# iosefa/obia

Measured on AMD Instinct MI355X. Metric: Mpixel/s (SLIC+zonal feats) on 16384²×8-band; achieved HBM GB/s fraction, higher is better.
Workload: dtype f32

## Files before the change

obia_amd/_lib.py:

```python
import ctypes
import os
import subprocess

import numpy as np

_CSRC = os.path.join(os.path.dirname(os.path.abspath(__file__)), "csrc")
LIB_PATH = os.environ.get("OBIA_HIP_LIB") or os.path.join(_CSRC, "libobia_hip.so")

OBIA_OK = 0
MASK_SEEDS_CHUNK = 1024
E_INVALID, E_HIP, E_NOMEM, E_UNSUPPORTED, E_EMPTY, E_NONFINITE = -1, -2, -3, -4, -5, -6


class SlicParams(ctypes.Structure):
    _fields_ = [("compactness", ctypes.c_double), ("min_size_factor", ctypes.c_double),
                ("max_size_factor", ctypes.c_double), ("n_segments", ctypes.c_int32),
                ("max_num_iter", ctypes.c_int32), ("convert2lab", ctypes.c_int32),
                ("enforce_connectivity", ctypes.c_int32), ("slic_zero", ctypes.c_int32),
                ("start_label", ctypes.c_int32), ("normalize_bands", ctypes.c_int32),
                ("exit_on_fixed_point", ctypes.c_int32), ("reserved", ctypes.c_int32),
                ("sigma_zyx", ctypes.c_double * 3), ("spacing_zyx", ctypes.c_double * 3)]


class SlicSeeds(ctypes.Structure):
# ... 140 lines not shown


def last_error():
    return load().obia_last_error().decode("utf-8", "replace")


def check(rc):
    if rc == OBIA_OK:
        return
    msg = last_error()
    if rc in (E_INVALID, E_EMPTY, E_NONFINITE):
        raise ValueError(msg)
    if rc == E_UNSUPPORTED:
        raise NotImplementedError(msg)
    if rc == E_NOMEM:
        raise MemoryError(msg)
    raise RuntimeError(f"obia_hip error {rc}: {msg}")


class Context:

    def __init__(self, device=0, stream=None):
        lib = load()
        if stream is None:
            self._h = lib.obia_create(int(device))
        else:
            self._h = lib.obia_create_on_stream(int(device), ctypes.c_void_p(int(stream)))
        if not self._h:
            raise RuntimeError(f"obia_create failed: {last_error()} (obia_amd needs an AMD GPU; there is no CPU path)")
        self.device = int(device)

    @property
    def handle(self):
        return self._h

    def close(self):
        if getattr(self, "_h", None):
            load().obia_destroy(self._h)
            self._h = None

    def __del__(self):
        try:
            self.close()
        except Exception:
            pass

    def set_profiling(self, on):
        check(load().obia_set_profiling(self._h, int(on)))

    def timing(self):
        lib = load()
        names = ["assign_ms", "sweeps", "features_ms", "connectivity_ms", "zonal_ms", "total_ms", "prepass_ms", "assign_px",
                 "prepass_px", "assign_store_px", "assign_busy_ms", "prepass_busy_ms", "batch_repeats",
                 "prepass_shared_px", "feature_fused_px"]
        return {n: lib.obia_last_timing(self._h, i) for i, n in enumerate(names)}

    def workspace_bytes(self):
        return int(load().obia_workspace_bytes(self._h))


_default_ctx = {}


def default_context(device=0):
    ctx = _default_ctx.get(device)
    if ctx is None:
        ctx = _default_ctx[device] = Context(device)
    return ctx


def np_ptr(a):
    return None if a is None else ctypes.c_void_p(a.ctypes.data)


def mask_bytes(mask, device=None):
    import torch
    m = torch.as_tensor(mask, device=device)
    if m.dtype == torch.bool:
        m = m.contiguous().view(torch.uint8)
    elif m.dtype != torch.uint8:
        m = (m != 0).view(torch.uint8)
    return m.contiguous()
```

obia_amd/csrc/common.hpp:

```cpp
#pragma once
#include <hip/hip_runtime.h>
#include <cstdint>
#include <cstdio>
#include <cstring>
#include <string>
#include <vector>

#include "../../include/obia_hip.h"

namespace obia {

void set_error(const char *fmt, ...);

#define OBIA_HIP_TRY(expr)                                                                       \
    do {                                                                                         \
        hipError_t e__ = (expr);                                                                 \
        if (e__ != hipSuccess) {                                                                 \
            obia::set_error("%s:%d: %s -> %s", __FILE__, __LINE__, #expr, hipGetErrorString(e__)); \
            return OBIA_E_HIP;                                                                   \
        }                                                                                        \
    } while (0)

#define OBIA_TRY(expr)            \
    do {                          \
        int rc__ = (expr);        \
        if (rc__ != OBIA_OK) return rc__; \
    } while (0)

class Arena {
  public:
    ~Arena() { release(); }
    void *alloc(size_t bytes);
    template <typename T> T *get(size_t n) { return static_cast<T *>(alloc(n * sizeof(T))); }
    void reset();
    void release();
    struct Mark { size_t block, used, total; };
    Mark mark() const;
    void rewind(const Mark &m);
    size_t capacity() const;
    bool failed() const { return failed_; }

  private:
    struct Block { char *p; size_t size; size_t used; };
    std::vector<Block> blocks_;
    size_t high_water_ = 0, cur_total_ = 0, cur_ = 0;
    bool failed_ = false;
};

struct Timing {
    double assign_ms = 0, prepass_ms = 0, feat_ms = 0, cc_ms = 0, zonal_ms = 0, total_ms = 0;
    double assign_px = 0, prepass_px = 0;
    double prepass_shared_px = 0;
    double assign_store_px = 0;
    double feat_fused_px = 0;
    int sweeps = 0;
    int batch_repeats = 0;
    double assign_busy_ms = 0, prepass_busy_ms = 0;
};

}

struct obia_ctx {
    int device = 0;
    hipStream_t stream = nullptr;
    bool own_stream = false;
    obia::Arena arena;
    void *pinned = nullptr;
    size_t pinned_bytes = 0;
    unsigned long long *defer_buf = nullptr;
    bool defer_pending = false;
    double defer_shared_px = 0;
    int32_t *cc_visited = nullptr;
    size_t cc_visited_px = 0;
    bool cc_visited_dirty = false;
    char *up_buf = nullptr;
    size_t up_bytes = 0, up_used = 0;
    int profiling = 0;
    obia::Timing timing;
    struct Span { int kind; hipEvent_t a, b; };
    std::vector<Span> spans;
    std::vector<hipEvent_t> event_pool;
    size_t events_used = 0;
    hipStream_t side = nullptr;
    hipEvent_t aux_fork = nullptr, aux_join = nullptr;
};

namespace obia {

enum TimeKind { T_ASSIGN = 0, T_FEAT = 2, T_CC = 3, T_ZONAL = 4, T_TOTAL = 5, T_PREPASS = 6 };

struct ScopedSpan {
    obia_ctx *ctx; bool on; size_t idx;
    ScopedSpan(obia_ctx *c, int kind);
    ~ScopedSpan();
};
struct KernelSpan {
    hipEvent_t a = nullptr, b = nullptr;
    KernelSpan(obia_ctx *c, int kind);
};
void begin_timing(obia_ctx *ctx);
void resolve_timing(obia_ctx *ctx);

int read_back(obia_ctx *ctx, void *host_dst, const void *dev_src, size_t bytes);
int upload_async(obia_ctx *ctx, void *dev_dst, const void *host_src, size_t bytes);
int side_stream(obia_ctx *ctx);
void debug_sync(obia_ctx *ctx, const char *stage);

static inline int cdiv(long long a, long long b) { return (int)((a + b - 1) / b); }

#if defined(__HIPCC__)
typedef float obia_v4f __attribute__((ext_vector_type(4)));
__device__ __forceinline__ float4 ld_stream_f4(const void *p) {
    const obia_v4f t = __builtin_nontemporal_load(reinterpret_cast<const obia_v4f *>(p));
    return make_float4(t.x, t.y, t.z, t.w);
}
#endif

}
```

obia_amd/csrc/context.cpp:

```cpp
#include "common.hpp"

#include <algorithm>
#include <cstdlib>
#include <utility>

#include <cstdarg>

namespace obia {

static thread_local std::string g_last_error;

void set_error(const char *fmt, ...) {
    char buf[1024];
    va_list ap;
    va_start(ap, fmt);
    vsnprintf(buf, sizeof(buf), fmt, ap);
    va_end(ap);
    g_last_error = buf;
}

void *Arena::alloc(size_t bytes) {
    bytes = (bytes + 255) & ~size_t(255);
    if (bytes == 0) bytes = 256;
    for (; cur_ < blocks_.size(); ++cur_) {
// ... 42 lines not shown
}

void Arena::reset() {
    failed_ = false;
    cur_total_ = 0;
    cur_ = 0;
    if (blocks_.size() > 1) {
        size_t total = 0;
        for (auto &b : blocks_) total += b.size;
        for (auto &b : blocks_) (void)hipFree(b.p);
        blocks_.clear();
        void *p = nullptr;
        if (hipMalloc(&p, high_water_ + (high_water_ >> 3)) == hipSuccess) blocks_.push_back(Block{static_cast<char *>(p), high_water_ + (high_water_ >> 3), 0});
        (void)total;
    } else if (!blocks_.empty()) {
        blocks_[0].used = 0;
    }
}

void Arena::release() {
    for (auto &b : blocks_) (void)hipFree(b.p);
    blocks_.clear();
}

size_t Arena::capacity() const {
    size_t t = 0;
    for (auto &b : blocks_) t += b.size;
    return t;
}

static hipEvent_t get_event(obia_ctx *ctx) {
    if (ctx->events_used == ctx->event_pool.size()) {
        hipEvent_t e = nullptr;
        (void)hipEventCreate(&e);
        ctx->event_pool.push_back(e);
    }
    return ctx->event_pool[ctx->events_used++];
}

ScopedSpan::ScopedSpan(obia_ctx *c, int kind) : ctx(c), on(c->profiling == 1 || (c->profiling == 2 && kind == T_ASSIGN)), idx(0) {
    if (!on) return;
    obia_ctx::Span s{kind, get_event(ctx), get_event(ctx)};
    (void)hipEventRecord(s.a, ctx->stream);
    idx = ctx->spans.size();
    ctx->spans.push_back(s);
}
ScopedSpan::~ScopedSpan() {
    if (on) (void)hipEventRecord(ctx->spans[idx].b, ctx->stream);
}

int side_stream(obia_ctx *ctx) {
    if (!ctx->aux_fork) OBIA_HIP_TRY(hipEventCreateWithFlags(&ctx->aux_fork, hipEventDisableTiming));
    if (!ctx->aux_join) OBIA_HIP_TRY(hipEventCreateWithFlags(&ctx->aux_join, hipEventDisableTiming));
    if (!ctx->side) OBIA_HIP_TRY(hipStreamCreateWithFlags(&ctx->side, hipStreamNonBlocking));
    return OBIA_OK;
}

KernelSpan::KernelSpan(obia_ctx *c, int kind) {
    if (!(c->profiling == 1 || (c->profiling == 2 && kind == T_ASSIGN))) return;
    a = get_event(c);
    b = get_event(c);
    c->spans.push_back(obia_ctx::Span{kind, a, b});
}

void begin_timing(obia_ctx *ctx) {
    ctx->spans.clear();
    ctx->events_used = 0;
    ctx->timing = Timing();
}

void resolve_timing(obia_ctx *ctx) {
    if (!ctx->profiling) return;
    (void)hipStreamSynchronize(ctx->stream);
    std::vector<std::pair<double, double>> iv[2];
    hipEvent_t ref = nullptr;
    for (auto &s : ctx->spans) {
        float ms = 0;
        if (hipEventElapsedTime(&ms, s.a, s.b) != hipSuccess) { (void)hipGetLastError(); continue; }
        if (s.kind == T_ASSIGN || s.kind == T_PREPASS) {
            if (!ref) ref = s.a;
            float end = 0;
            if (hipEventElapsedTime(&end, ref, s.b) == hipSuccess) iv[s.kind == T_ASSIGN ? 0 : 1].emplace_back((double)end - ms, (double)end);
            else (void)hipGetLastError();
        }
        switch (s.kind) {
            case T_ASSIGN: ctx->timing.assign_ms += ms; ctx->timing.sweeps += 1; break;
            case T_FEAT: ctx->timing.feat_ms += ms; break;
            case T_CC: ctx->timing.cc_ms += ms; break;
            case T_ZONAL: ctx->timing.zonal_ms += ms; break;
            case T_TOTAL: ctx->timing.total_ms += ms; break;
            case T_PREPASS: ctx->timing.prepass_ms += ms; break;
            default: break;
        }
    }
    for (int c = 0; c < 2; ++c) {
        std::sort(iv[c].begin(), iv[c].end());
        double busy = 0, lo = 0, hi = -1;
        for (auto &x : iv[c]) {
            if (hi < lo || x.first > hi) { if (hi > lo) busy += hi - lo; lo = x.first; hi = x.second; }
            else if (x.second > hi) hi = x.second;
        }
        if (hi > lo) busy += hi - lo;
        (c == 0 ? ctx->timing.assign_busy_ms : ctx->timing.prepass_busy_ms) += busy;
    }
    ctx->spans.clear();
}
// ... 53 lines not shown
using namespace obia;

extern "C" {

int obia_abi_version(void) { return OBIA_ABI_VERSION; }

const char *obia_last_error(void) { return g_last_error.c_str(); }

static obia_ctx *create_impl(int device_id, void *stream, bool own) {
    int n = 0;
    if (hipGetDeviceCount(&n) != hipSuccess || n <= 0) {
        set_error("no HIP device available");
        return nullptr;
    }
    if (device_id < 0 || device_id >= n) {
        set_error("device_id %d out of range (%d devices)", device_id, n);
        return nullptr;
    }
    if (hipSetDevice(device_id) != hipSuccess) {
        set_error("hipSetDevice(%d) failed", device_id);
        return nullptr;
    }
    obia_ctx *ctx = new obia_ctx();
    ctx->device = device_id;
    if (own) {
        if (hipStreamCreateWithFlags(&ctx->stream, hipStreamNonBlocking) != hipSuccess) {
            set_error("hipStreamCreate failed");
            delete ctx;
            return nullptr;
        }
        ctx->own_stream = true;
    } else {
        ctx->stream = static_cast<hipStream_t>(stream);
    }
    return ctx;
}

obia_ctx *obia_create(int device_id) { return create_impl(device_id, nullptr, true); }
obia_ctx *obia_create_on_stream(int device_id, void *hip_stream) { return create_impl(device_id, hip_stream, false); }

void obia_destroy(obia_ctx *ctx) {
    if (!ctx) return;
    (void)hipSetDevice(ctx->device);
    (void)hipStreamSynchronize(ctx->stream);
    ctx->arena.release();
    if (ctx->up_buf) (void)hipHostFree(ctx->up_buf);
    if (ctx->pinned) (void)hipHostFree(ctx->pinned);
    if (ctx->defer_buf) (void)hipHostFree(ctx->defer_buf);
    if (ctx->cc_visited) (void)hipFree(ctx->cc_visited);
    for (auto e : ctx->event_pool) (void)hipEventDestroy(e);
    if (ctx->side) (void)hipStreamDestroy(ctx->side);
    if (ctx->aux_fork) (void)hipEventDestroy(ctx->aux_fork);
    if (ctx->aux_join) (void)hipEventDestroy(ctx->aux_join);
    if (ctx->own_stream) (void)hipStreamDestroy(ctx->stream);
    delete ctx;
}

int obia_synchronize(obia_ctx *ctx) {
    if (!ctx) { set_error("null context"); return OBIA_E_INVALID; }
    OBIA_HIP_TRY(hipStreamSynchronize(ctx->stream));
    return OBIA_OK;
}

int64_t obia_workspace_bytes(obia_ctx *ctx) { return ctx ? (int64_t)ctx->arena.capacity() : 0; }

void obia_slic_default_params(obia_slic_params *p) {
    if (!p) return;
    p->n_segments = 100;
    p->compactness = 10.0;
    p->max_num_iter = 10;
    p->convert2lab = -1;
    p->enforce_connectivity = 1;
    p->min_size_factor = 0.5;
    p->max_size_factor = 3.0;
    p->slic_zero = 0;
    p->start_label = 1;
    p->normalize_bands = 0;
    p->exit_on_fixed_point = 0;
    p->reserved = 0;
    p->sigma_zyx[0] = p->sigma_zyx[1] = p->sigma_zyx[2] = 0.0;
    p->spacing_zyx[0] = p->spacing_zyx[1] = p->spacing_zyx[2] = 1.0;
}

int obia_set_profiling(obia_ctx *ctx, int enabled) {
    if (!ctx) { set_error("null context"); return OBIA_E_INVALID; }
    ctx->profiling = enabled < 0 ? 0 : (enabled > 2 ? 1 : enabled);
    return OBIA_OK;
}

double obia_last_timing(obia_ctx *ctx, int what) {
    if (!ctx) return -1.0;
    switch (what) {
        case 0: return ctx->timing.assign_ms;
        case 1: return (double)ctx->timing.sweeps;
        case 2: return ctx->timing.feat_ms;
        case 3: return ctx->timing.cc_ms;
        case 4: return ctx->timing.zonal_ms;
        case 5: return ctx->timing.total_ms;
        case 6: return ctx->timing.prepass_ms;
        case 7: return ctx->timing.assign_px;
        case 8: return ctx->timing.prepass_px;
        case 9: return ctx->timing.assign_store_px;
        case 10: return ctx->timing.assign_busy_ms;
        case 11: return ctx->timing.prepass_busy_ms;
        case 12: return (double)ctx->timing.batch_repeats;
        case 13: return ctx->timing.prepass_shared_px;
        case 14: return ctx->timing.feat_fused_px;
        default: return -1.0;
    }
}

}
```

obia_amd/csrc/slic_sweep.hip:

```cpp
#include "slic.hpp"
#include "slic_features.hpp"

#include <type_traits>
#include <hip/hip_ext.h>

#include <cstdlib>

namespace obia {

#ifdef OBIA_STAMP
__device__ unsigned long long g_tl[65536 * 4 * 24];
#define STAMP_DECL unsigned long long st_t = clock64(), st_t0 = st_t, st_r0 = __builtin_amdgcn_s_memrealtime(), st_acc[12] = {0, 0, 0, 0, 0, 0, 0, 0, 0, 0, 0, 0}, st_cnt[6] = {0, 0, 0, 0, 0, 0};
#define STAMP_COUNT(i, v) st_cnt[i] += (v);
#define STAMP(i) { const unsigned long long st_n = clock64(); st_acc[i] += st_n - st_t; st_t = st_n; }
#ifndef OBIA_STAMP_KIND
#define OBIA_STAMP_KIND 0
#endif
#define STAMP_FLUSH if (accumulate && (LEAN ? 1 : 0) == OBIA_STAMP_KIND && (threadIdx.x & 63) == 0 && gtile < 65536) { unsigned long long *st_o = g_tl + ((size_t)gtile * 4 + (threadIdx.x >> 6)) * 24; for (int st_i = 0; st_i < 12; ++st_i) st_o[st_i] = st_acc[st_i]; st_o[12] = st_t0; st_o[13] = clock64(); st_o[14] = st_r0; st_o[15] = __builtin_amdgcn_s_memrealtime(); for (int st_i = 0; st_i < 6; ++st_i) st_o[16 + st_i] = st_cnt[st_i]; }
#else
#define STAMP_DECL
#define STAMP(i)
#define STAMP_COUNT(i, v)
#define STAMP_FLUSH
#endif
// ... 86 lines not shown
        if (live) a[q] = 0ull;
        const unsigned long long nq = __shfl(aq, gl0 + CP);
        const unsigned long long syq = __shfl(aq, gl0 + CP + 1);
        const unsigned long long sxq = __shfl(aq, gl0 + CP + 2);
        const float fn = (float)nq;
        cy = (float)syq / fn;
        cx = (float)sxq / fn;
        bool mq = false;
        if (live && q < CP) {
            const float sum = (float)((double)(long long)aq * inv_fscale);
            const float v = sum / fn;
            mq = __float_as_uint(v) != __float_as_uint(oldc);
            rec[CENT_REC + q] = v;
        }
        const unsigned long long mb = __ballot(mq);
        const unsigned long long gmask = (G == 64) ? ~0ull : (((1ull << G) - 1ull) << gl0);
        moved = (mb & gmask) != 0ull;
        moved |= __float_as_uint(cy) != __float_as_uint(old_cy) || __float_as_uint(cx) != __float_as_uint(old_cx);
    }
    if (!live || q != 0) return;
    const float mdc = slic_zero ? ((first || slic_zero == 2) ? 1.0f : rec[7]) : 0.0f;
    if (bin_stamp && moved && !first && old_cy == old_cy && old_cx == old_cx) {
        int oby = (int)(old_cy / (float)P.sy), obx = (int)(old_cx / (float)P.sx);
        oby = oby < 0 ? 0 : (oby >= P.ncy ? P.ncy - 1 : oby);
        obx = obx < 0 ? 0 : (obx >= P.ncx ? P.ncx - 1 : obx);
        bin_stamp[P.cell_off + oby * P.ncx + obx] = sweep_id;
    }
    float4 *hrec = reinterpret_cast<float4 *>(rec);
    if (!(cy == cy) || !(cx == cx)) {
        hrec[0] = make_float4(cy, cx, 0.0f, 0.0f);
        hrec[1] = make_float4(0.0f, 0.0f, __int_as_float(-1), mdc);
        return;
    }
    float fy0 = cy - (float)(2 * P.sy); fy0 = (0.0f > fy0) ? 0.0f : fy0;
    float fy1 = (cy + (float)(2 * P.sy)) + 1.0f; fy1 = ((float)P.H < fy1) ? (float)P.H : fy1;
    float fx0 = cx - (float)(2 * P.sx); fx0 = (0.0f > fx0) ? 0.0f : fx0;
    float fx1 = (cx + (float)(2 * P.sx)) + 1.0f; fx1 = ((float)P.W < fx1) ? (float)P.W : fx1;
    int by = (int)(cy / (float)P.sy), bx = (int)(cx / (float)P.sx);
    by = by < 0 ? 0 : (by >= P.ncy ? P.ncy - 1 : by);
    bx = bx < 0 ? 0 : (bx >= P.ncx ? P.ncx - 1 : bx);
    const int link = atomicExch(&head[P.cell_off + by * P.ncx + bx], k);
    hrec[0] = make_float4(cy, cx, __int_as_float((int)fy0), __int_as_float((int)fy1));
    hrec[1] = make_float4(__int_as_float((int)fx0), __int_as_float((int)fx1), __int_as_float(link), mdc);
    if (bin_stamp && moved) bin_stamp[P.cell_off + by * P.ncx + bx] = sweep_id;
    list_margin_check(P, k, cy, cx, (int)fy0, (int)fy1, (int)fx0, (int)fx1, first != 0, ref, tl_req, sweep_id);
}

template <int CP>
__global__ __launch_bounds__(64) void slic_prep_lane_kernel(const SlicProblem *__restrict__ probs, int p_base,
                                                             int first, int slic_zero, const float *__restrict__ seed,
                                                             unsigned long long *__restrict__ acc, int RQ, double inv_fscale,
                                                             float *__restrict__ cent, int *__restrict__ head,
                                                             int *__restrict__ head_other,
                                                             int total_cells, int *__restrict__ bin_stamp, int sweep_id,
                                                             int cell_base, float *__restrict__ ref, int *__restrict__ tl_req,
                                                             const int *__restrict__ act_probs) {
    constexpr int RS = CENT_REC + CP;
    constexpr int NQ = (CP + 3 + 1) / 2;
    {
        const int nthr = gridDim.x * gridDim.y * blockDim.x;
        for (int i = cell_base + (blockIdx.y * gridDim.x + blockIdx.x) * blockDim.x + threadIdx.x; i < total_cells; i += nthr) head_other[i] = -1;
    }
    const SlicProblem P = probs[act_probs ? act_probs[blockIdx.y] : p_base + (int)blockIdx.y];
    const int kl = blockIdx.x * blockDim.x + threadIdx.x;
    if (kl >= P.K) return;
    const int k = P.cent_off + kl;
    float4 *hrec = reinterpret_cast<float4 *>(cent + (size_t)k * RS);
    ulonglong2 *a2 = reinterpret_cast<ulonglong2 *>(acc + (size_t)k * RQ);
    const float4 h0 = hrec[0], h1 = hrec[1];
    float4 oc[CP / 4];
    ulonglong2 aq[NQ];
    if (!first) {
        if (bin_stamp) {
#pragma unroll
            for (int i = 0; i < CP / 4; ++i) oc[i] = hrec[2 + i];
        } else {
#pragma unroll
            for (int i = 0; i < CP / 4; ++i) oc[i] = make_float4(0.f, 0.f, 0.f, 0.f);
        }
#pragma unroll
        for (int i = 0; i < NQ; ++i) aq[i] = a2[i];
    }
    const float old_cy = h0.x, old_cx = h0.y;
    float cy, cx;
    bool moved;
    if (first) {
        cy = seed[2 * (size_t)k];
        cx = seed[2 * (size_t)k + 1];
#pragma unroll
        for (int i = 0; i < CP / 4; ++i) hrec[2 + i] = make_float4(0.0f, 0.0f, 0.0f, 0.0f);
        moved = true;
    } else {
        unsigned long long q[2 * NQ];
#pragma unroll
        for (int i = 0; i < NQ; ++i) { q[2 * i] = aq[i].x; q[2 * i + 1] = aq[i].y; a2[i] = make_ulonglong2(0ull, 0ull); }
        const float fn = (float)(double)q[CP];
        cy = (float)(double)q[CP + 1] / fn;
        cx = (float)(double)q[CP + 2] / fn;
        moved = false;
        float nc[CP];
#pragma unroll
        for (int ch = 0; ch < CP; ++ch) {
            const float sum = (float)((double)(long long)q[ch] * inv_fscale);
            nc[ch] = sum / fn;
        }
#pragma unroll
        for (int i = 0; i < CP / 4; ++i) {
            moved |= __float_as_uint(nc[4 * i]) != __float_as_uint(oc[i].x) || __float_as_uint(nc[4 * i + 1]) != __float_as_uint(oc[i].y)
                  || __float_as_uint(nc[4 * i + 2]) != __float_as_uint(oc[i].z) || __float_as_uint(nc[4 * i + 3]) != __float_as_uint(oc[i].w);
            hrec[2 + i] = make_float4(nc[4 * i], nc[4 * i + 1], nc[4 * i + 2], nc[4 * i + 3]);
        }
        moved |= __float_as_uint(cy) != __float_as_uint(old_cy) || __float_as_uint(cx) != __float_as_uint(old_cx);
    }
    const float mdc = slic_zero ? ((first || slic_zero == 2) ? 1.0f : h1.w) : 0.0f;
// ... 896 lines not shown
    slic_assign_body<CP, MASKED, false, false, false, false, true, NCH>(OBIA_ASSIGN_ARGS, nullptr);
}

template <int CP, bool MASKED, bool FIXPT>
__global__ __launch_bounds__(NT) __attribute__((amdgpu_waves_per_eu(LEAN_WAVES, LEAN_WAVES))) void slic_prepass_kernel(OBIA_ASSIGN_PARAMS, const int *__restrict__ act_tiles) {
    slic_assign_body<CP, MASKED, true, FIXPT, false, true, false>(OBIA_ASSIGN_ARGS, act_tiles);
}

#include "slic_spatial.hip"

#ifdef OBIA_STAMP
extern "C" void obia_debug_timeline(unsigned long long *out, int nwaves) {
    (void)hipMemcpyFromSymbol(out, HIP_SYMBOL(g_tl), sizeof(unsigned long long) * 24 * (size_t)nwaves);
}
#endif

template <int CP, bool MASKED>
__global__ __launch_bounds__(256) void slic_maxdist_kernel(const SlicProblem *__restrict__ probs, const float *__restrict__ feat,
                                                           const uint8_t *__restrict__ mask, const int32_t *__restrict__ labels,
                                                           float *__restrict__ cent, int start_label, int nch) {
    constexpr int RS = CENT_REC + CP;
    const SlicProblem P = probs[blockIdx.y];
    for (int y = blockIdx.x; y < P.H; y += gridDim.x)
        for (int x = threadIdx.x; x < P.W; x += 256) {
            const long long pix = P.pix_off + (long long)y * P.W + x;
            if (MASKED && mask[pix] == 0) continue;
            const int l = labels[pix];
            if (l < start_label) continue;
            const int k = l - start_label + P.cent_off;
            const float *rec = cent + (size_t)k * RS;
            float dc = 0.0f;
#pragma unroll
            for (int ch = 0; ch < CP; ++ch) {
                if (ch >= nch) break;
                const float t = feat_at(feat, P, CP, y, x, ch) - rec[CENT_REC + ch];
                dc += t * t;
            }
            unsigned *slot = reinterpret_cast<unsigned *>(cent + (size_t)k * RS + 7);
            if (__float_as_uint(dc) > __hip_atomic_load(slot, __ATOMIC_RELAXED, __HIP_MEMORY_SCOPE_AGENT)) atomicMax(slot, __float_as_uint(dc));
        }
}

struct TileSubset { const int *table = nullptr; int base = 0, end = -1; };

struct FixedPointState {
    int *bin_stamp = nullptr, *tile_lp = nullptr, *cache_k = nullptr;
    unsigned long long *cache_q = nullptr;
};

template <int CP>
static void launch_assign(obia_ctx *ctx, SlicBatch &b, int ignore_color, int accumulate, int accum_color, int store_labels,
                          int *orphan_flag, const FixedPointState &fp, int sweep_id, int use_cache, unsigned long long *px_counter,
                          const KernelSpan &span, const int *head_cur, bool prepass_visits, const TileSubset &sub = TileSubset(),
                          bool rawin = false) {
    constexpr int XGH = OBIA_XCD_GROUP;
    const int ntiles = sub.end >= 0 ? sub.end : (int)b.total_tiles_all, tbase = sub.end >= 0 ? sub.base : 0;
    dim3 grid(8 * XGH * (unsigned)((ntiles - tbase + 8 * XGH - 1) / (8 * XGH)));
    const int RQ = acc_record_qwords(CP);
    int tpp = b.probs.empty() ? 0 : b.probs[0].tiles_x * b.probs[0].tiles_y;
    for (auto &P : b.probs) if (P.tiles_x * P.tiles_y != tpp) tpp = 0;
#define LAUNCH_ARGS_                                                                                                 \
    b.d_probs, b.d_feat, b.d_mask, b.d_mask4, b.d_cent, head_cur, b.d_labels, b.d_acc, RQ, accumulate, store_labels, b.start_label,      \
        (float)b.fscale, fp.bin_stamp, fp.tile_lp, fp.cache_k, fp.cache_q, sweep_id, use_cache, px_counter,          \
        b.d_tile_prob, ntiles, orphan_flag, tpp, b.d_fbox, tbase, b.C, b.d_tl_k, b.d_tl_fp, b.d_tl_meta, b.d_tl_req
#define LAUNCH_K_(...)                                                                                               \
    hipExtLaunchKernelGGL(HIP_KERNEL_NAME(__VA_ARGS__), grid, dim3(NT), 0, ctx->stream, span.a, span.b, 0, LAUNCH_ARGS_)
#define LAUNCH_KL_(...)                                                                                              \
    hipExtLaunchKernelGGL(HIP_KERNEL_NAME(__VA_ARGS__), grid, dim3(NT), 0, ctx->stream, span.a, span.b, 0, LAUNCH_ARGS_, sub.table)
    const int pad = CP - b.C;
    if constexpr (CP <= 12) if (rawin) {
        RawInput ri;
        ri.src = b.raw_src; ri.Ws = b.raw_ws; ri.wins = b.d_windows; ri.keys = b.d_keys; ri.ratio = b.feat_ratio; ri.planes = b.d_feat;
        hipExtLaunchKernelGGL(HIP_KERNEL_NAME(slic_assign_rawin_kernel<CP>), grid, dim3(NT), 0, ctx->stream, span.a, span.b, 0, LAUNCH_ARGS_, ri);
        ctx->timing.feat_fused_px += (double)b.total_pix;
        return;
    }
#define LAUNCH_ASSIGN_(M, I, F, Z) LAUNCH_K_(slic_assign_kernel<CP, M, I, F, Z>)
#define LAUNCH_MAIN_(M)                                                                                              \
    do {                                                                                                             \
        if (pad == 1) LAUNCH_K_(slic_assign_kernel<CP, M, false, false, false, CP - 1>);                             \
        else if (pad == 2) LAUNCH_K_(slic_assign_kernel<CP, M, false, false, false, CP - 2>);                        \
        else if (pad == 3) LAUNCH_K_(slic_assign_kernel<CP, M, false, false, false, CP - 3>);                        \
        else LAUNCH_K_(slic_assign_kernel<CP, M, false, false, false>);                                              \
    } while (0)
#define LAUNCH_COLLB_(M)                                                                                             \
    do {                                                                                                             \
        if (pad == 1) LAUNCH_K_(slic_assign_collb_kernel<CP, M, CP - 1>);                                            \
        else if (pad == 2) LAUNCH_K_(slic_assign_collb_kernel<CP, M, CP - 2>);                                       \
        else if (pad == 3) LAUNCH_K_(slic_assign_collb_kernel<CP, M, CP - 3>);                                       \
        else LAUNCH_K_(slic_assign_collb_kernel<CP, M>);                                                             \
    } while (0)
#define LAUNCH_LEAN_(M, F) LAUNCH_KL_(slic_prepass_kernel<CP, M, F>)
#define LAUNCH_ASSIGN(M, I)                                                                                          \
    do {                                                                                                             \
        if ((I) && !accum_color) {                                                                                   \
            if (fp.bin_stamp) LAUNCH_LEAN_(M, true);                                                                 \
            else if (store_labels || prepass_visits) LAUNCH_LEAN_(M, false);                                         \
            else LAUNCH_KL_(slic_spatial_kernel<CP>);                                                                \
        }                                                                                                            \
        else if (b.slic_zero && !(I)) LAUNCH_ASSIGN_(M, false, false, true);                                         \
        else if (fp.bin_stamp) LAUNCH_ASSIGN_(M, I, true, false);                                                    \
        else if (b.col_lb && b.d_fbox && !(I)) LAUNCH_COLLB_(M);                                                     \
        else if (!(I)) LAUNCH_MAIN_(M);                                                                              \
        else LAUNCH_ASSIGN_(M, I, false, false);                                                                     \
    } while (0)
    if (b.masked) { if (ignore_color) LAUNCH_ASSIGN(true, true); else LAUNCH_ASSIGN(true, false); }
    else LAUNCH_ASSIGN(false, false);
#undef LAUNCH_ASSIGN
#undef LAUNCH_ASSIGN_
#undef LAUNCH_LEAN_
#undef LAUNCH_COLLB_
#undef LAUNCH_MAIN_
#undef LAUNCH_K_
#undef LAUNCH_KL_
#undef LAUNCH_ARGS_
}

__global__ __launch_bounds__(256) void mask_pack4_kernel(const SlicProblem *__restrict__ probs, const uint8_t *__restrict__ mask,
                                                         unsigned *__restrict__ mask4) {
    const SlicProblem P = probs[blockIdx.y];
    if ((long long)P.n_valid == (long long)P.H * (long long)P.W) return;
    const int nq = (P.H + 3) >> 2, W = P.W;
    const uint8_t *mb = mask + P.pix_off;
    unsigned *out = mask4 + P.m4_off;
    const bool vec = (W % 4 == 0) && (P.pix_off % 4 == 0) && (P.m4_off % 4 == 0) && (reinterpret_cast<uintptr_t>(mask) % 4 == 0) &&
                     (reinterpret_cast<uintptr_t>(mask4) % 16 == 0);
// ... 1 lines not shown
        if (vec) {
            for (int x4 = threadIdx.x; x4 < (W >> 2); x4 += 256) {
                unsigned r[4];
#pragma unroll
                for (int j = 0; j < 4; ++j) {
                    const int y = 4 * q + j;
                    r[j] = y < P.H ? *reinterpret_cast<const unsigned *>(mb + (long long)y * W + 4 * x4) : 0u;
                }
                uint4 o;
                unsigned *ov = &o.x;
#pragma unroll
                for (int c = 0; c < 4; ++c) {
                    unsigned w = 0u;
#pragma unroll
                    for (int j = 0; j < 4; ++j) w |= (unsigned)(((r[j] >> (8 * c)) & 0xffu) != 0u) << (8 * j);
                    ov[c] = w;
                }
                *reinterpret_cast<uint4 *>(out + (long long)q * W + 4 * x4) = o;
            }
        } else {
            for (int x = threadIdx.x; x < W; x += 256) {
                unsigned w = 0u;
#pragma unroll
                for (int j = 0; j < 4; ++j) {
                    const int y = 4 * q + j;
                    if (y < P.H) w |= (unsigned)(mb[(long long)y * W + x] != 0) << (8 * j);
                }
                out[(long long)q * W + x] = w;
            }
        }
    }
}

__global__ void fill_i32_kernel(int32_t *p, long long n, int32_t v) {
    for (long long i = (long long)blockIdx.x * blockDim.x + threadIdx.x; i < n; i += (long long)gridDim.x * blockDim.x) p[i] = v;
}

static void fill_labels(obia_ctx *ctx, SlicBatch &b) {
    const long long n = b.total_pix;
    int blocks = cdiv(n, 256 * 8);
    if (blocks > 65535) blocks = 65535;
    if (blocks < 1) blocks = 1;
    hipLaunchKernelGGL(fill_i32_kernel, dim3(blocks), dim3(256), 0, ctx->stream, b.d_labels, n, b.start_label - 1);
}

static void fold_counters(obia_ctx *ctx, const unsigned long long *h, double shared_px) {
    if (ctx->profiling) {
        for (int i = 0; i < 256; ++i) { ctx->timing.assign_px += (double)h[i]; ctx->timing.prepass_px += (double)h[256 + i]; }
        ctx->timing.prepass_px += shared_px;
        ctx->timing.prepass_shared_px += shared_px;
    }
}

static int queue_sweeps(obia_ctx *ctx, SlicBatch &b, bool repeat, unsigned long long **d_px_out, double *shared_px_out) {
    *d_px_out = nullptr;
    *shared_px_out = 0.0;
    if (std::getenv("OBIA_DEBUG_SYNC"))
        for (size_t p = 0; p < b.probs.size(); ++p) {
            const SlicProblem &P = b.probs[p];
            fprintf(stderr, "[obia debug]   problem %zu: %dx%d K %d steps %d %d bins %dx%d cell_off %d cent_off %d tiles %dx%d tile_off %d n_valid %d (total_cent %d total_cells %d tiles_all %lld)\n",
                    p, P.H, P.W, P.K, P.sy, P.sx, P.ncy, P.ncx, P.cell_off, P.cent_off, P.tiles_y, P.tiles_x, P.tile_off, P.n_valid,
                    b.total_cent, b.total_cells, b.total_tiles_all);
        }
    if (b.total_tiles <= 0 || b.max_iter <= 0) { fill_labels(ctx, b); return OBIA_OK; }
    for (auto &P : b.probs)
        if (P.W >= (1 << 22)) { set_error("rasters / tile windows wider than 4194303 pixels are not supported (got %d)", P.W); return OBIA_E_UNSUPPORTED; }
    const int passes = (b.masked && !b.prepass_only) ? 2 : 1;
    if (b.fuse_features && (!b.masked || b.exit_on_fixed_point || b.slic_zero || b.direct || b.col_lb || b.C != b.CP || b.CP > 12 || !b.raw_src || !b.d_keys)) {
        set_error("fused feature pass on a batch that cannot take it");
        return OBIA_E_INVALID;
    }
    const int pre_iter = (b.masked && b.prepass_iter > 0) ? b.prepass_iter : b.max_iter;
    const int total_sweeps = b.masked ? pre_iter + (passes - 1) * b.max_iter : b.max_iter;
    const int RQ = acc_record_qwords(b.CP);
    Arena &A = ctx->arena;
    unsigned long long *d_px = A.get<unsigned long long>(513);
    if (!d_px) return OBIA_E_NOMEM;
    int *d_orphan = reinterpret_cast<int *>(d_px + 512);
    FixedPointState fp;
    if (b.exit_on_fixed_point) {
        const size_t nt = (size_t)b.total_tiles_all;
        fp.bin_stamp = A.get<int>((size_t)b.total_cells);
        fp.tile_lp = A.get<int>(nt);
        fp.cache_k = A.get<int>(nt * (MAXC + 1));
        fp.cache_q = A.get<unsigned long long>(nt * MAXC * (size_t)(b.CP + 3));
        if (!fp.bin_stamp || !fp.tile_lp || !fp.cache_k || !fp.cache_q) return OBIA_E_NOMEM;
        OBIA_HIP_TRY(hipMemsetAsync(fp.bin_stamp, 0, sizeof(int) * (size_t)b.total_cells, ctx->stream));
        OBIA_HIP_TRY(hipMemsetAsync(fp.tile_lp, 0, sizeof(int) * nt, ctx->stream));
    }
    {
        const size_t nt = (size_t)b.total_tiles_all;
        b.d_tl_k = A.get<int>(nt * MAXC);
        b.d_tl_fp = A.get<unsigned>(nt * NT);
        b.d_tl_meta = A.get<int>(nt * 3);
        b.d_tl_req = b.d_tl_meta ? b.d_tl_meta + nt * 2 : nullptr;
        b.d_ref = A.get<float>((size_t)b.total_cent * 2);
        if (!b.d_tl_k || !b.d_tl_fp || !b.d_tl_meta || !b.d_tl_req || !b.d_ref) return OBIA_E_NOMEM;
    }
    int maxh_z = 1, kmax = 1;
    for (auto &P : b.probs) { if (P.H > maxh_z) maxh_z = P.H; if (P.K > kmax) kmax = P.K; }
    if (b.masked && b.d_mask && !b.d_mask4) {
        b.d_mask4 = A.get<unsigned>((size_t)b.total_m4);
        if (!b.d_mask4) return OBIA_E_NOMEM;
        int gq = (maxh_z + 3) / 4;
        if (gq > 16384) gq = 16384;
        hipLaunchKernelGGL(mask_pack4_kernel, dim3(gq, b.nprob), dim3(256), 0, ctx->stream, b.d_probs, b.d_mask, b.d_mask4);
// ... 6 lines not shown
        debug_sync(ctx, "sweeps: label fill");
    }
    if (repeat) OBIA_HIP_TRY(hipMemsetAsync(b.d_acc, 0, sizeof(unsigned long long) * (size_t)b.total_cent * RQ, ctx->stream));
    const bool prep_grouped = std::getenv("OBIA_PREP_GROUPED") != nullptr;
    const bool prepass_visits = std::getenv("OBIA_PREPASS_VISITS") != nullptr;
    std::vector<int> share_rep;
    int n_shared = 0;
    {
        const char *e = std::getenv("OBIA_PREPASS_SHARE");
        const bool off = e && e[0] == '0';
        if (!off && b.masked && passes == 2 && pre_iter >= 2 && b.prepass_iter <= 0 && !store_all && !b.direct && !prep_grouped)
            n_shared = slic_prepass_classes(b.probs, b.grid_n, share_rep);
    }
    TileSubset act_tiles;
    const int *d_act_probs = nullptr;
    const int *d_member_rep = nullptr;
    int act_p_base = 0, n_act = b.nprob, kmax_act = kmax, kmax_mem = 1;
    if (n_shared > 0) {
        std::vector<int> ap, at, mr;
        double spx = 0.0;
        kmax_act = 1;
        for (int p = 0; p < b.nprob; ++p) {
            const SlicProblem &P = b.probs[p];
            if (share_rep[p] == p) {
                ap.push_back(p);
                for (int t = 0; t < P.tiles_x * P.tiles_y; ++t) at.push_back(P.tile_off + t);
                if (P.K > kmax_act) kmax_act = P.K;
            } else {
                mr.push_back(p); mr.push_back(share_rep[p]);
                if (P.K > kmax_mem) kmax_mem = P.K;
                spx += (double)P.H * (double)P.W * (double)(pre_iter - 1);
            }
        }
        n_act = (int)ap.size();
        act_p_base = ap.front();
        const bool span = ap.back() - ap.front() + 1 == n_act;
        int *d_mr = A.get<int>(mr.size());
        if (!d_mr) return OBIA_E_NOMEM;
        OBIA_TRY(upload_async(ctx, d_mr, mr.data(), sizeof(int) * mr.size()));
        d_member_rep = d_mr;
        if (span) {
            act_tiles.base = b.probs[ap.front()].tile_off;
            act_tiles.end = b.probs[ap.back()].tile_off + b.probs[ap.back()].tiles_x * b.probs[ap.back()].tiles_y;
        } else {
            int *d_ap = A.get<int>(ap.size()), *d_at = A.get<int>(at.size() ? at.size() : 1);
            if (!d_ap || !d_at) return OBIA_E_NOMEM;
            OBIA_TRY(upload_async(ctx, d_ap, ap.data(), sizeof(int) * ap.size()));
            if (!at.empty()) OBIA_TRY(upload_async(ctx, d_at, at.data(), sizeof(int) * at.size()));
            d_act_probs = d_ap;
            act_tiles.table = d_at; act_tiles.base = 0; act_tiles.end = (int)at.size();
        }
        *shared_px_out = spx;
    }
    OBIA_HIP_TRY(hipMemsetAsync(d_px, 0, sizeof(unsigned long long) * 513, ctx->stream));
    OBIA_HIP_TRY(hipMemsetAsync(b.d_head, 0xff, sizeof(int) * (size_t)b.total_cells, ctx->stream));
    OBIA_HIP_TRY(hipMemsetAsync(b.d_tl_meta, 0xff, sizeof(int) * 3 * (size_t)b.total_tiles_all, ctx->stream));
    debug_sync(ctx, "sweeps: memsets");
    bool first = true;
    int sweep_no = 0;
    for (int pass = 0; pass < passes; ++pass) {
        const int ignore_color = (b.masked && pass == 0) ? 1 : 0;
        const bool last_pass = (pass == passes - 1);
        if (pass > 0 && store_all) {
            fill_labels(ctx, b);
            if (fp.tile_lp) OBIA_HIP_TRY(hipMemsetAsync(fp.tile_lp, 0, sizeof(int) * (size_t)b.total_tiles_all, ctx->stream));
        }
        const int iters = ignore_color ? pre_iter : b.max_iter;
        for (int it = 0; it < iters; ++it) {
            int *head_cur = b.d_head + (size_t)(sweep_no & 1) * b.total_cells;
            int *head_nxt = b.d_head + (size_t)((sweep_no + 1) & 1) * b.total_cells;
            ++sweep_no;
            const int zmode = (b.slic_zero && !ignore_color) ? (it == 0 ? 2 : 1) : 0;
            const bool shared_sweep = n_shared > 0 && ignore_color && it < iters - 1;
            if (n_shared > 0 && ignore_color && it == iters - 1) {
                hipLaunchKernelGGL(slic_prepass_broadcast_kernel, dim3(cdiv(kmax_mem, 64), n_shared), dim3(64), 0, ctx->stream, b.d_probs,
                                   d_member_rep, b.CP, RQ, b.d_acc, b.d_cent, b.d_ref);
                debug_sync(ctx, "sweeps: pre-pass broadcast");
            }
            const dim3 prep_grid(cdiv(shared_sweep ? kmax_act : kmax, 64), shared_sweep ? n_act : b.nprob);
            const int prep_base = shared_sweep ? act_p_base : 0;
            const int *prep_table = shared_sweep ? d_act_probs : nullptr;
#define LAUNCH_PREP_LANE(CPV)                                                                                         \
    hipLaunchKernelGGL(HIP_KERNEL_NAME(slic_prep_lane_kernel<CPV>), prep_grid, dim3(64), 0, ctx->stream, \
                       b.d_probs, prep_base, first ? 1 : 0, zmode, b.d_seed, b.d_acc, RQ, 1.0 / b.fscale, b.d_cent, head_cur, head_nxt, \
                       b.total_cells, fp.bin_stamp, sweep_no, 0, b.d_ref, b.d_tl_req, prep_table)
            if (!prep_grouped) {
                switch (b.CP) {
                    case 4: LAUNCH_PREP_LANE(4); break;
                    case 8: LAUNCH_PREP_LANE(8); break;
                    case 12: LAUNCH_PREP_LANE(12); break;
                    default: LAUNCH_PREP_LANE(16); break;
                }
            } else if (RQ == 16)
                hipLaunchKernelGGL(HIP_KERNEL_NAME(slic_prep_kernel<16>), dim3(cdiv(b.total_cent * 16LL, 256)), dim3(256), 0,
                                   ctx->stream, b.d_probs, b.d_cent_prob, b.total_cent, b.CP, first ? 1 : 0, zmode, b.d_seed, b.d_acc,
                                   1.0 / b.fscale, b.d_cent, head_cur, head_nxt, b.total_cells, fp.bin_stamp, sweep_no, 0, 0, b.d_ref, b.d_tl_req);
            else
                hipLaunchKernelGGL(HIP_KERNEL_NAME(slic_prep_kernel<32>), dim3(cdiv(b.total_cent * 32LL, 256)), dim3(256), 0,
                                   ctx->stream, b.d_probs, b.d_cent_prob, b.total_cent, b.CP, first ? 1 : 0, zmode, b.d_seed, b.d_acc,
                                   1.0 / b.fscale, b.d_cent, head_cur, head_nxt, b.total_cells, fp.bin_stamp, sweep_no, 0, 0, b.d_ref, b.d_tl_req);
#undef LAUNCH_PREP_LANE
            b.d_head_cur = head_cur;
            debug_sync(ctx, "sweeps: prep");
            first = false;
            if (zmode == 1) {
                dim3 zg(maxh_z, b.nprob);
#define LAUNCH_MAXDIST(CPV)                                                                                           \
    do {                                                                                                              \
        if (b.masked) hipLaunchKernelGGL(HIP_KERNEL_NAME(slic_maxdist_kernel<CPV, true>), zg, dim3(256), 0, ctx->stream, b.d_probs, \
                                         b.d_feat, b.d_mask, b.d_labels, b.d_cent, b.start_label, b.C);            \
        else hipLaunchKernelGGL(HIP_KERNEL_NAME(slic_maxdist_kernel<CPV, false>), zg, dim3(256), 0, ctx->stream, b.d_probs, \
                                b.d_feat, b.d_mask, b.d_labels, b.d_cent, b.start_label, b.C);                     \
    } while (0)
                switch (b.CP) {
                    case 4: LAUNCH_MAXDIST(4); break;
                    case 8: LAUNCH_MAXDIST(8); break;
                    case 12: LAUNCH_MAXDIST(12); break;
                    default: LAUNCH_MAXDIST(16); break;
                }
#undef LAUNCH_MAXDIST
            }
            const bool very_last = last_pass && it == iters - 1;
            const int accumulate = very_last ? 0 : 1;
            const int accum_color = (!ignore_color || it == iters - 1) ? 1 : 0;
            const int store_labels = store_all ? 2 : (very_last ? 1 : 0);
            const int use_cache = (ignore_color && it == iters - 1) ? 0 : 1;
            const bool rawin = b.fuse_features && !repeat && ignore_color && it == iters - 1;
            {
                KernelSpan span(ctx, ignore_color ? T_PREPASS : T_ASSIGN);
                const TileSubset sub = shared_sweep ? act_tiles : TileSubset();
                unsigned long long *pxc = ctx->profiling ? d_px + (ignore_color ? 256 : 0) : nullptr;
                if (ctx->profiling && !ignore_color && store_labels) ctx->timing.assign_store_px += (double)b.total_pix;
                switch (b.CP) {
                    case 8: launch_assign<8>(ctx, b, ignore_color, accumulate, accum_color, store_labels, d_orphan, fp, sweep_no, use_cache, pxc, span, head_cur, prepass_visits, sub, rawin); break;
#ifndef OBIA_ONLY_CP8
                    case 4: launch_assign<4>(ctx, b, ignore_color, accumulate, accum_color, store_labels, d_orphan, fp, sweep_no, use_cache, pxc, span, head_cur, prepass_visits, sub, rawin); break;
                    case 12: launch_assign<12>(ctx, b, ignore_color, accumulate, accum_color, store_labels, d_orphan, fp, sweep_no, use_cache, pxc, span, head_cur, prepass_visits, sub, rawin); break;
                    case 16: launch_assign<16>(ctx, b, ignore_color, accumulate, accum_color, store_labels, d_orphan, fp, sweep_no, use_cache, pxc, span, head_cur, prepass_visits, sub); break;
#endif
                    default: set_error("bad CP"); return OBIA_E_INVALID;
                }
            }
            debug_sync(ctx, ignore_color ? "sweeps: pre-pass sweep" : "sweeps: colour sweep");
        }
    }
    OBIA_HIP_TRY(hipGetLastError());
    *d_px_out = d_px;
    return OBIA_OK;
}

int slic_run_sweeps(obia_ctx *ctx, SlicBatch &b) {
    ctx->defer_pending = false;
    unsigned long long *d_px = nullptr;
    ctx->defer_shared_px = 0.0;
// ... 32 lines not shown
```

Baseline: 7237.

## Split masked pre-pass sweeps into two problem groups on concurrent streams

During masked pre-pass sweeps, the problems are split into two groups with roughly equal tile counts. Each group's prep and assign kernels run on its own stream (main and side), so one group can advance to its next sweep without waiting for the other to finish. The split is skipped when the smaller group has fewer tiles than the device can keep resident, and it can be turned off with an environment variable. This adds event fork/join handling and a second stream, and it relies on the two groups' cell and tile ranges being disjoint.

```diff
diff --git a/obia_amd/_lib.py b/obia_amd/_lib.py
--- a/obia_amd/_lib.py
+++ b/obia_amd/_lib.py
@@ -216,7 +216,7 @@
         lib = load()
         names = ["assign_ms", "sweeps", "features_ms", "connectivity_ms", "zonal_ms", "total_ms", "prepass_ms", "assign_px",
                  "prepass_px", "assign_store_px", "assign_busy_ms", "prepass_busy_ms", "batch_repeats",
-                 "prepass_shared_px", "feature_fused_px"]
+                 "prepass_shared_px", "feature_fused_px", "prepass_group_launches"]
         return {n: lib.obia_last_timing(self._h, i) for i, n in enumerate(names)}
 
     def workspace_bytes(self):
diff --git a/obia_amd/csrc/common.hpp b/obia_amd/csrc/common.hpp
--- a/obia_amd/csrc/common.hpp
+++ b/obia_amd/csrc/common.hpp
@@ -54,6 +54,7 @@
     double assign_store_px = 0;
     double feat_fused_px = 0;
     int sweeps = 0;
+    int prepass_group_launches = 0;
     int batch_repeats = 0;
     double assign_busy_ms = 0, prepass_busy_ms = 0;
 };
@@ -83,6 +84,8 @@
     size_t events_used = 0;
     hipStream_t side = nullptr;
     hipEvent_t aux_fork = nullptr, aux_join = nullptr;
+    hipEvent_t grp_fork = nullptr, grp_join = nullptr;
+    int spatial_residency[4] = {0, 0, 0, 0};
 };
 
 namespace obia {
diff --git a/obia_amd/csrc/context.cpp b/obia_amd/csrc/context.cpp
--- a/obia_amd/csrc/context.cpp
+++ b/obia_amd/csrc/context.cpp
@@ -118,6 +118,8 @@
 int side_stream(obia_ctx *ctx) {
     if (!ctx->aux_fork) OBIA_HIP_TRY(hipEventCreateWithFlags(&ctx->aux_fork, hipEventDisableTiming));
     if (!ctx->aux_join) OBIA_HIP_TRY(hipEventCreateWithFlags(&ctx->aux_join, hipEventDisableTiming));
+    if (!ctx->grp_fork) OBIA_HIP_TRY(hipEventCreateWithFlags(&ctx->grp_fork, hipEventDisableTiming));
+    if (!ctx->grp_join) OBIA_HIP_TRY(hipEventCreateWithFlags(&ctx->grp_join, hipEventDisableTiming));
     if (!ctx->side) OBIA_HIP_TRY(hipStreamCreateWithFlags(&ctx->side, hipStreamNonBlocking));
     return OBIA_OK;
 }
@@ -277,6 +279,8 @@
     if (ctx->side) (void)hipStreamDestroy(ctx->side);
     if (ctx->aux_fork) (void)hipEventDestroy(ctx->aux_fork);
     if (ctx->aux_join) (void)hipEventDestroy(ctx->aux_join);
+    if (ctx->grp_fork) (void)hipEventDestroy(ctx->grp_fork);
+    if (ctx->grp_join) (void)hipEventDestroy(ctx->grp_join);
     if (ctx->own_stream) (void)hipStreamDestroy(ctx->stream);
     delete ctx;
 }
@@ -331,6 +335,7 @@
         case 12: return (double)ctx->timing.batch_repeats;
         case 13: return ctx->timing.prepass_shared_px;
         case 14: return ctx->timing.feat_fused_px;
+        case 15: return (double)ctx->timing.prepass_group_launches;
         default: return -1.0;
     }
 }
diff --git a/obia_amd/csrc/slic_sweep.hip b/obia_amd/csrc/slic_sweep.hip
--- a/obia_amd/csrc/slic_sweep.hip
+++ b/obia_amd/csrc/slic_sweep.hip
@@ -162,14 +162,14 @@
                                                              unsigned long long *__restrict__ acc, int RQ, double inv_fscale,
                                                              float *__restrict__ cent, int *__restrict__ head,
                                                              int *__restrict__ head_other,
-                                                             int total_cells, int *__restrict__ bin_stamp, int sweep_id,
+                                                             int cell_end, int *__restrict__ bin_stamp, int sweep_id,
                                                              int cell_base, float *__restrict__ ref, int *__restrict__ tl_req,
                                                              const int *__restrict__ act_probs) {
     constexpr int RS = CENT_REC + CP;
     constexpr int NQ = (CP + 3 + 1) / 2;
     {
         const int nthr = gridDim.x * gridDim.y * blockDim.x;
-        for (int i = cell_base + (blockIdx.y * gridDim.x + blockIdx.x) * blockDim.x + threadIdx.x; i < total_cells; i += nthr) head_other[i] = -1;
+        for (int i = cell_base + (blockIdx.y * gridDim.x + blockIdx.x) * blockDim.x + threadIdx.x; i < cell_end; i += nthr) head_other[i] = -1;
     }
     const SlicProblem P = probs[act_probs ? act_probs[blockIdx.y] : p_base + (int)blockIdx.y];
     const int kl = blockIdx.x * blockDim.x + threadIdx.x;
@@ -1172,7 +1172,8 @@
 static void launch_assign(obia_ctx *ctx, SlicBatch &b, int ignore_color, int accumulate, int accum_color, int store_labels,
                           int *orphan_flag, const FixedPointState &fp, int sweep_id, int use_cache, unsigned long long *px_counter,
                           const KernelSpan &span, const int *head_cur, bool prepass_visits, const TileSubset &sub = TileSubset(),
-                          bool rawin = false) {
+                          bool rawin = false, const hipStream_t *on = nullptr) {
+    const hipStream_t stream = on ? *on : ctx->stream;
     constexpr int XGH = OBIA_XCD_GROUP;
     const int ntiles = sub.end >= 0 ? sub.end : (int)b.total_tiles_all, tbase = sub.end >= 0 ? sub.base : 0;
     dim3 grid(8 * XGH * (unsigned)((ntiles - tbase + 8 * XGH - 1) / (8 * XGH)));
@@ -1184,14 +1185,14 @@
         (float)b.fscale, fp.bin_stamp, fp.tile_lp, fp.cache_k, fp.cache_q, sweep_id, use_cache, px_counter,          \
         b.d_tile_prob, ntiles, orphan_flag, tpp, b.d_fbox, tbase, b.C, b.d_tl_k, b.d_tl_fp, b.d_tl_meta, b.d_tl_req
 #define LAUNCH_K_(...)                                                                                               \
-    hipExtLaunchKernelGGL(HIP_KERNEL_NAME(__VA_ARGS__), grid, dim3(NT), 0, ctx->stream, span.a, span.b, 0, LAUNCH_ARGS_)
+    hipExtLaunchKernelGGL(HIP_KERNEL_NAME(__VA_ARGS__), grid, dim3(NT), 0, stream, span.a, span.b, 0, LAUNCH_ARGS_)
 #define LAUNCH_KL_(...)                                                                                              \
-    hipExtLaunchKernelGGL(HIP_KERNEL_NAME(__VA_ARGS__), grid, dim3(NT), 0, ctx->stream, span.a, span.b, 0, LAUNCH_ARGS_, sub.table)
+    hipExtLaunchKernelGGL(HIP_KERNEL_NAME(__VA_ARGS__), grid, dim3(NT), 0, stream, span.a, span.b, 0, LAUNCH_ARGS_, sub.table)
     const int pad = CP - b.C;
     if constexpr (CP <= 12) if (rawin) {
         RawInput ri;
         ri.src = b.raw_src; ri.Ws = b.raw_ws; ri.wins = b.d_windows; ri.keys = b.d_keys; ri.ratio = b.feat_ratio; ri.planes = b.d_feat;
-        hipExtLaunchKernelGGL(HIP_KERNEL_NAME(slic_assign_rawin_kernel<CP>), grid, dim3(NT), 0, ctx->stream, span.a, span.b, 0, LAUNCH_ARGS_, ri);
+        hipExtLaunchKernelGGL(HIP_KERNEL_NAME(slic_assign_rawin_kernel<CP>), grid, dim3(NT), 0, stream, span.a, span.b, 0, LAUNCH_ARGS_, ri);
         ctx->timing.feat_fused_px += (double)b.total_pix;
         return;
     }
@@ -1299,6 +1300,26 @@
     }
 }
 
+static int spatial_residency(obia_ctx *ctx, int CP) {
+    int &r = ctx->spatial_residency[CP / 4 - 1];
+    if (r > 0) return r;
+    int per_cu = 0, cus = 0;
+    hipError_t e = hipErrorInvalidValue;
+    switch (CP) {
+        case 8: e = hipOccupancyMaxActiveBlocksPerMultiprocessor(&per_cu, slic_spatial_kernel<8>, NT, 0); break;
+#ifndef OBIA_ONLY_CP8
+        case 4: e = hipOccupancyMaxActiveBlocksPerMultiprocessor(&per_cu, slic_spatial_kernel<4>, NT, 0); break;
+        case 12: e = hipOccupancyMaxActiveBlocksPerMultiprocessor(&per_cu, slic_spatial_kernel<12>, NT, 0); break;
+        case 16: e = hipOccupancyMaxActiveBlocksPerMultiprocessor(&per_cu, slic_spatial_kernel<16>, NT, 0); break;
+#endif
+        default: break;
+    }
+    if (e == hipSuccess) e = hipDeviceGetAttribute(&cus, hipDeviceAttributeMultiprocessorCount, ctx->device);
+    if (e != hipSuccess || per_cu <= 0 || cus <= 0) { (void)hipGetLastError(); return 0x7fffffff; }
+    r = per_cu * cus;
+    return r;
+}
+
 static int queue_sweeps(obia_ctx *ctx, SlicBatch &b, bool repeat, unsigned long long **d_px_out, double *shared_px_out) {
     *d_px_out = nullptr;
     *shared_px_out = 0.0;
@@ -1411,6 +1432,24 @@
         }
         *shared_px_out = spx;
     }
+    int grp_split = 0;
+    {
+        const char *e = std::getenv("OBIA_PREPASS_GROUPS");
+        const int mode = !e ? 1 : (e[0] == '0' ? 0 : (e[0] == '2' ? 2 : 1));
+        if (mode != 0 && n_shared == 0 && b.masked && pre_iter >= 2 && !store_all && !prepass_visits && !prep_grouped && !b.direct &&
+            b.nprob >= 2 && !std::getenv("OBIA_DEBUG_SYNC")) {
+            long long best = -1;
+            for (int p = 1; p < b.nprob; ++p) {
+                const long long t0 = b.probs[p].tile_off, t1 = b.total_tiles_all - t0, d = t0 > t1 ? t0 - t1 : t1 - t0;
+                if (t0 > 0 && t1 > 0 && (best < 0 || d <= best)) { best = d; grp_split = p; }
+            }
+            if (grp_split > 0 && mode != 2) {
+                const long long t0 = b.probs[grp_split].tile_off, t1 = b.total_tiles_all - t0;
+                if ((t0 < t1 ? t0 : t1) < (long long)spatial_residency(ctx, b.CP)) grp_split = 0;
+            }
+            if (grp_split > 0) OBIA_TRY(side_stream(ctx));
+        }
+    }
     OBIA_HIP_TRY(hipMemsetAsync(d_px, 0, sizeof(unsigned long long) * 513, ctx->stream));
     OBIA_HIP_TRY(hipMemsetAsync(b.d_head, 0xff, sizeof(int) * (size_t)b.total_cells, ctx->stream));
     OBIA_HIP_TRY(hipMemsetAsync(b.d_tl_meta, 0xff, sizeof(int) * 3 * (size_t)b.total_tiles_all, ctx->stream));
@@ -1440,17 +1479,61 @@
             const int prep_base = shared_sweep ? act_p_base : 0;
             const int *prep_table = shared_sweep ? d_act_probs : nullptr;
 #define LAUNCH_PREP_LANE(CPV)                                                                                         \
-    hipLaunchKernelGGL(HIP_KERNEL_NAME(slic_prep_lane_kernel<CPV>), prep_grid, dim3(64), 0, ctx->stream, \
-                       b.d_probs, prep_base, first ? 1 : 0, zmode, b.d_seed, b.d_acc, RQ, 1.0 / b.fscale, b.d_cent, head_cur, head_nxt, \
-                       b.total_cells, fp.bin_stamp, sweep_no, 0, b.d_ref, b.d_tl_req, prep_table)
-            if (!prep_grouped) {
+    hipLaunchKernelGGL(HIP_KERNEL_NAME(slic_prep_lane_kernel<CPV>), pgrid, dim3(64), 0, stream, \
+                       b.d_probs, p_base, first ? 1 : 0, zmode, b.d_seed, b.d_acc, RQ, 1.0 / b.fscale, b.d_cent, head_cur, head_nxt, \
+                       cell_end, fp.bin_stamp, sweep_no, cell_base, b.d_ref, b.d_tl_req, table)
+            auto prep_lane = [&](hipStream_t stream, dim3 pgrid, int p_base, const int *table, int cell_base, int cell_end) {
                 switch (b.CP) {
                     case 4: LAUNCH_PREP_LANE(4); break;
                     case 8: LAUNCH_PREP_LANE(8); break;
                     case 12: LAUNCH_PREP_LANE(12); break;
                     default: LAUNCH_PREP_LANE(16); break;
                 }
-            } else if (RQ == 16)
+            };
+#undef LAUNCH_PREP_LANE
+            if (grp_split > 0 && ignore_color && it < iters - 1) {
+                hipError_t he = hipSuccess;
+                if (it == 0) {
+                    he = hipEventRecord(ctx->grp_fork, ctx->stream);
+                    if (he == hipSuccess) he = hipStreamWaitEvent(ctx->side, ctx->grp_fork, 0);
+                }
+                for (int g = 0; g < 2 && he == hipSuccess; ++g) {
+                    const int p0 = g ? grp_split : 0, p1 = g ? b.nprob : grp_split;
+                    int kmax_g = 1;
+                    for (int p = p0; p < p1; ++p) if (b.probs[p].K > kmax_g) kmax_g = b.probs[p].K;
+                    const hipStream_t st = g ? ctx->side : ctx->stream;
+                    prep_lane(st, dim3(cdiv(kmax_g, 64), p1 - p0), p0, nullptr, b.probs[p0].cell_off, g ? b.total_cells : b.probs[p1].cell_off);
+                    KernelSpan span(ctx, T_PREPASS);
+                    TileSubset sub;
+                    sub.base = b.probs[p0].tile_off;
+                    sub.end = g ? (int)b.total_tiles_all : b.probs[p1].tile_off;
+                    unsigned long long *pxc = ctx->profiling ? d_px + 256 : nullptr;
+                    switch (b.CP) {
+                        case 8: launch_assign<8>(ctx, b, 1, 1, 0, 0, d_orphan, fp, sweep_no, 1, pxc, span, head_cur, false, sub, false, &st); break;
+#ifndef OBIA_ONLY_CP8
+                        case 4: launch_assign<4>(ctx, b, 1, 1, 0, 0, d_orphan, fp, sweep_no, 1, pxc, span, head_cur, false, sub, false, &st); break;
+                        case 12: launch_assign<12>(ctx, b, 1, 1, 0, 0, d_orphan, fp, sweep_no, 1, pxc, span, head_cur, false, sub, false, &st); break;
+                        case 16: launch_assign<16>(ctx, b, 1, 1, 0, 0, d_orphan, fp, sweep_no, 1, pxc, span, head_cur, false, sub, false, &st); break;
+#endif
+                        default: he = hipErrorInvalidValue; break;
+                    }
+                    ctx->timing.prepass_group_launches += 1;
+                }
+                if (he == hipSuccess && it == iters - 2) {
+                    he = hipEventRecord(ctx->grp_join, ctx->side);
+                    if (he == hipSuccess) he = hipStreamWaitEvent(ctx->stream, ctx->grp_join, 0);
+                }
+                if (he != hipSuccess) {
+                    (void)hipStreamSynchronize(ctx->side);
+                    set_error("grouped pre-pass: %s", hipGetErrorString(he));
+                    return OBIA_E_HIP;
+                }
+                b.d_head_cur = head_cur;
+                first = false;
+                continue;
+            }
+            if (!prep_grouped) prep_lane(ctx->stream, prep_grid, prep_base, prep_table, 0, b.total_cells);
+            else if (RQ == 16)
                 hipLaunchKernelGGL(HIP_KERNEL_NAME(slic_prep_kernel<16>), dim3(cdiv(b.total_cent * 16LL, 256)), dim3(256), 0,
                                    ctx->stream, b.d_probs, b.d_cent_prob, b.total_cent, b.CP, first ? 1 : 0, zmode, b.d_seed, b.d_acc,
                                    1.0 / b.fscale, b.d_cent, head_cur, head_nxt, b.total_cells, fp.bin_stamp, sweep_no, 0, 0, b.d_ref, b.d_tl_req);
@@ -1458,7 +1541,6 @@
                 hipLaunchKernelGGL(HIP_KERNEL_NAME(slic_prep_kernel<32>), dim3(cdiv(b.total_cent * 32LL, 256)), dim3(256), 0,
                                    ctx->stream, b.d_probs, b.d_cent_prob, b.total_cent, b.CP, first ? 1 : 0, zmode, b.d_seed, b.d_acc,
                                    1.0 / b.fscale, b.d_cent, head_cur, head_nxt, b.total_cells, fp.bin_stamp, sweep_no, 0, 0, b.d_ref, b.d_tl_req);
-#undef LAUNCH_PREP_LANE
             b.d_head_cur = head_cur;
             debug_sync(ctx, "sweeps: prep");
             first = false;
```

Result: faster. 7388 (median of 6 runs) (+2.1%).
